# sevagh/Zen

Measured on AMD Instinct MI355X. Metric: hops/sec (1024-hop HPR, 44.1 kHz mono), higher is better.
Workload: dtype f32

## Files before the change

zen_amd/blockrun/blockrun.hip:

```cpp
#include "../csrc/hpr_engine.h"
#include "../csrc/masks.h"
#include "blockrun_first_pass.h"
#include "blockrun_kernel.h"
#include "zen_hip_blockrun.h"

#include <atomic>
#include <cstring>
#include <vector>

using namespace zen_hip_impl;

namespace {

std::atomic<int> g_run_len{0}, g_min_items{4096}, g_off{0};
std::atomic<unsigned long long> g_routed{0}, g_forwarded{0};

struct ProfScope {
	zen_hip_hpr* e;
	int k;
	hipEvent_t e0 = nullptr, e1 = nullptr;
	ProfScope(zen_hip_hpr* e_, int k_)
	    : e(e_)
	    , k(k_)
	{
		if (!e->prof)
			return;
		if (!e->prof_pool.empty()) {
			e0 = e->prof_pool.back().first;
			e1 = e->prof_pool.back().second;
			e->prof_pool.pop_back();
		}
		else if (hipEventCreate(&e0) != hipSuccess || hipEventCreate(&e1) != hipSuccess) {
			e0 = e1 = nullptr;
			return;
		}
		(void)hipEventRecord(e0, e->stream);
	}
	~ProfScope()
	{
		if (!e0)
			return;
		(void)hipEventRecord(e1, e->stream);
		e->prof_pending.push_back({k, e0, e1});
		e->prof_launches[k] += 1;
	}
};

int device_slots(int* slots)
{
	static std::atomic<int> cached[64];
	int dev = 0;
	ZH_HIP(hipGetDevice(&dev));
	int v = (dev >= 0 && dev < 64) ? cached[dev].load() : 0;
	if (v == 0) {
		int cus = 0;
		ZH_HIP(hipDeviceGetAttribute(&cus, hipDeviceAttributeMultiprocessorCount, dev));
		v = 3 * (cus > 0 ? cus : 1);
		if (dev >= 0 && dev < 64)
			cached[dev].store(v);
	}
	*slots = v;
	return ZEN_HIP_OK;
}

struct FirstPassTable {
	int symmetric;
	float2 tw16, tw8, tw3_16;
};
const FirstPassTable& first_pass_table()
{
	static const FirstPassTable t = [] {
		constexpr int n = zen_blockrun::NFFT;
		std::vector<float> tw(n);
		make_twiddles(tw.data(), tw.size());
		FirstPassTable r;
		r.symmetric = zen_blockrun::table_is_symmetric(tw.data(), n) ? 1 : 0;
		r.tw16 = make_float2(tw[2 * (n / 16)], tw[2 * (n / 16) + 1]);
		r.tw8 = make_float2(tw[2 * (n / 8)], tw[2 * (n / 8) + 1]);
		r.tw3_16 = make_float2(tw[2 * (3 * n / 16)], tw[2 * (3 * n / 16) + 1]);
		return r;
	}();
	return t;
}

bool takes(const zen_hip_hpr* h, const float* in, size_t n_hops, size_t in_stride, const float* harm, const float* perc,
           const float* resid, size_t out_stride)
{
	if (g_off.load() || !h || !in || !perc || harm || resid || n_hops == 0)
		return false;
	if (h->causality != ZEN_HIP_TIME_CAUSAL || h->log2n != 12 || h->mf != zen_blockrun::TAPS || h->hop != (size_t)zen_blockrun::HOP
	    || h->nfft != (size_t)zen_blockrun::NFFT || h->nwin != 2 * h->hop)
		return false;
	if (!h->out_p || h->out_h || h->out_r || h->soft || h->use_sse)
		return false;
	if ((h->drain[0] | h->drain[1] | h->drain[2]) || h->rows_stale || h->run_mode || h->res_idle_ms != 0 || h->res_active || h->dbg_stamps)
		return false;
	if (!h->d_Y[0] || !h->d_blk_need || !h->d_carry[0] || !h->d_mag || n_hops > h->max_hops)
		return false;
	if (h->n_streams * n_hops < (size_t)g_min_items.load() || h->n_streams * n_hops > 0x3fffffffu)
		return false;
	int inc = 0;
	if (hard_mask_threshold(h->beta, &inc) == 0.0)
		return false;
	const size_t S = h->n_streams;
	const char *in0 = (const char*)in, *in1 = (const char*)(in + (S - 1) * in_stride + n_hops * h->hop);
	const char *o0 = (const char*)perc, *o1 = (const char*)(perc + (S - 1) * out_stride + n_hops * h->hop);
	return !(o0 < in1 && in0 < o1);
}

}

extern "C" int zen_hip_blockrun_process(zen_hip_hpr_t h, const float* in_dev, size_t n_hops, size_t in_stride, float* harm, float* perc,
                                        float* resid, size_t out_stride)
{
	if (!takes(h, in_dev, n_hops, in_stride, harm, perc, resid, out_stride)) {
		g_forwarded.fetch_add(1);
		return zen_hip_hpr_process(h, in_dev, n_hops, in_stride, harm, perc, resid, out_stride);
	}
	g_routed.fetch_add(1);
	int slots = 0;
	ZH_TRY(device_slots(&slots));
	zen_blockrun::RunArgs a;
	memset(&a, 0, sizeof(a));
	a.in = in_dev;
	a.in_stride = (long long)in_stride;
	a.tail_prev = h->d_tail[h->tail_sel];
	a.tail_next = h->d_tail[h->tail_sel ^ 1];
	a.window = h->d_window;
	a.tw = h->d_tw;
	{
		const FirstPassTable& t = first_pass_table();
		a.tw_symmetric = t.symmetric;
		a.tw16 = t.tw16;
		a.tw8 = t.tw8;
		a.tw3_16 = t.tw3_16;
	}
	a.mag = h->d_mag;
	a.keep_mag_rows = (int)h->W - 1;
	a.ring_rows = h->ring_rows;
	a.row0 = h->abs_frame;
	a.n_frames = (int)n_hops;
	a.n_streams = (int)h->n_streams;
	a.prev_frames = (int)h->last_frames;
	a.carry = h->d_carry[0];
	a.Y = h->d_Y[0];
	a.y_stream_stride = (long long)(h->max_hops * h->nwin);
	a.out = perc;
	a.out_stride = (long long)out_stride;
	a.need = h->d_blk_need;
	a.cola = h->cola;
	int inc = 0;
	a.thr = hard_mask_threshold(h->beta, &inc);
	a.part = zen_blockrun_partition(a.n_streams, a.n_frames, slots, g_run_len.load());
	for (int o = 0; o < 3; ++o) {
		h->ready_valid[o] = false;
		h->direct_done[o] = false;
	}
	{
		ProfScope ps(h, zen_hip_hpr::K_FUSED);
		ZH_TRY(zen_blockrun::launch_run(a, h->stream));
	}
	{
		ProfScope ps(h, zen_hip_hpr::K_FINALIZE);
		ZH_TRY(zen_blockrun::launch_fixup(a, h->stream));
	}
	h->tail_sel ^= 1;
	h->abs_frame += (long long)n_hops;
	h->last_frames = n_hops;
	return ZEN_HIP_OK;
}

extern "C" int zen_hip_blockrun_set(const char* key, int value)
{
	if (!key || value < 0)
		ZH_FAIL(ZEN_HIP_E_BAD_ARG, "blockrun_set: null key or negative value");
	if (!strcmp(key, "run_len"))
		g_run_len.store(value);
	else if (!strcmp(key, "min_items"))
		g_min_items.store(value);
	else if (!strcmp(key, "off"))
		g_off.store(value);
	else
		ZH_FAIL(ZEN_HIP_E_BAD_ARG, "blockrun_set: unknown key '%s' (run_len, min_items, off)", key);
	return ZEN_HIP_OK;
}

extern "C" int zen_hip_blockrun_stats(unsigned long long* routed, unsigned long long* forwarded)
{
	if (routed)
		*routed = g_routed.load();
	if (forwarded)
		*forwarded = g_forwarded.load();
	return ZEN_HIP_OK;
}
```

zen_amd/blockrun/blockrun_kernel.h:

```cpp
#pragma once
#include <hip/hip_runtime.h>

#include "blockrun_partition.h"

namespace zen_blockrun {

constexpr int HOP = 1024, NFFT = 4096, TAPS = 47;

struct RunArgs {
	const float* in;
	long long in_stride;
	const float* tail_prev;
	float* tail_next;
	const float* window;
	const float2* tw;
	int tw_symmetric;
	float2 tw16, tw8, tw3_16;
	float* mag;
	int keep_mag_rows;
	long long ring_rows, row0;
	int n_frames, n_streams, prev_frames;
	float* carry;
	float* Y;
	long long y_stream_stride;
	float* out;
	long long out_stride;
	unsigned* need;
	float cola;
	double thr;
	zen_blockrun_part part;
};

constexpr size_t LDS_BYTES_MAX = 53 * 1024;
size_t run_kernel_lds_bytes();
int launch_run(const RunArgs& a, hipStream_t stream);
int launch_fixup(const RunArgs& a, hipStream_t stream);

}
```

zen_amd/blockrun/blockrun_kernel.hip:

```cpp
#include "../csrc/common.h"
#include "../csrc/fft_dev.h"
#include "../csrc/masks.h"
#include "../csrc/median47_core.h"
#include "../csrc/median_net.h"
#include "blockrun_kernel.h"
#include "blockrun_first_pass.h"
#include "blockrun_edge_count.h"

#pragma clang fp contract(off)

namespace zen_blockrun {
namespace {

using zen_hip_impl::hard_mask_exact;
using PL = zfft::Plan<12>;
constexpr int N = PL::N, TF = PL::TF;
static_assert(N == NFFT && TF == 256 && HOP == 4 * TF, "four samples of a hop per thread");

constexpr int MID = TAPS / 2, MID_AL = 24, IMG_END = 255 * 16 + 64;
__device__ __forceinline__ int img_addr(int g) { return (g >> 4) * zm47::RSTR + (g & 15); }
constexpr int MIR_LO = 56, MIR_HI = 39;
static_assert(N - MIR_LO <= 16 * 254 - 24 && N / 2 + MIR_HI >= 16 * 128 + 39, "blocks 254 / 255 and 126 .. 128 read written columns");
static_assert(EDGE_IMG_COL0 == MID_AL && EDGE_IMG_RSTR == zm47::RSTR && EDGE_OUTPUTS == MID + 1, "blockrun_edge_count.h reads this image");
constexpr int PC_WORD = 5184, PC_TAIL = 2052, EDGE_WORD = PC_WORD + PC_TAIL + 512 + 4;
static_assert((EDGE_WORD + 256) * 4 <= PL::LDS_FLOAT2 * 8, "lean layout must fit in the frame image");
constexpr int KEEP_WORD = PL::LDS_FLOAT2 * 2, CARRY_WORD = KEEP_WORD + HOP, WIN_WORD = CARRY_WORD + HOP;
constexpr size_t LDS_BYTES = (size_t)(WIN_WORD + 2 * HOP) * 4;
static_assert(LDS_BYTES <= LDS_BYTES_MAX, "three workgroups per CU");

__device__ __forceinline__ void lds_barrier()
{
	asm volatile("s_waitcnt lgkmcnt(0)\n\ts_barrier" ::: "memory");
}

struct TwGlobal32 {
	static constexpr bool PLAIN = true;
	static constexpr bool PACKED = true;
	const float2* __restrict__ p;
	__device__ __forceinline__ float2 get(int, int, int, int idx) const
	{
		return *reinterpret_cast<const float2*>(reinterpret_cast<const char*>(p) + (unsigned)(idx << 3));
	}
};

struct Spec {
	float2 S[16];
};

struct FwdInPre {
	float x[8], w[8];
	__device__ __forceinline__ float2 operator()(int, int slot) const { return make_float2(x[slot] * w[slot], 0.0f); }
};

struct FwdOut {
	Spec* r;
	int* img;
	__device__ __forceinline__ void operator()(int idx, float2 X, bool lower, int slot) const
	{
		r->S[slot] = X;
		if (slot == 8) {
			if (__builtin_amdgcn_readfirstlane(idx) < (N >> 1) + 64 && idx == (N >> 1))
				img[img_addr((N >> 1) + MID_AL)] = __float_as_int(zfft::cabs_exact(X.x, X.y));
		}
		else if (lower) {
			const float m = zfft::cabs_exact(X.x, X.y);
			const int key = __float_as_int(m);
			constexpr int CH = (TF / 16) * zm47::RSTR;
			const int tfl = idx - slot * TF;
			img[img_addr(tfl + MID_AL) + slot * CH] = key;
			if (slot == 0 && tfl >= 1 && tfl <= MIR_LO)
				img[img_addr(N - tfl + MID_AL)] = key;
			if (slot == 7 && tfl >= TF - MIR_HI)
				img[img_addr(N - 7 * TF - tfl + MID_AL)] = key;
		}
	}
};

struct InvIn {
	const Spec* r;
	const int* img;
	const float* pc;
	double thr;
	__device__ __forceinline__ float2 operator()(int idx, int slot) const
	{
		const int lo = slot * TF, hi = lo + TF - 1;
		int pi;
		if (hi <= N / 2)
			pi = idx;
		else if (lo > N / 2 && hi < N - MID)
			pi = N - idx;
		else
			pi = (idx > N / 2 && idx < N - MID) ? N - idx : (idx > N / 2 ? idx - (N - 512) + PC_TAIL : idx);
		const int g0 = hi <= N / 2 ? idx + 24 - slot * TF : TF + 24 - (idx - slot * TF);
		const float mag = __int_as_float(img[(g0 >> 4) * 20 + (g0 & 15) + (hi <= N / 2 ? slot : 15 - slot) * (TF / 16) * 20]);
		const float2 z = r->S[slot];
		const float p = pc[pi];
		float m = hard_mask_exact(p, mag + FLT_EPSILON, thr);
		if (hi > N / 2 && !(lo > N / 2 && hi < N - MID))
			m = (idx == N / 2 || idx >= N - MID) ? p : m;
		return make_float2(z.x * m, z.y * m);
	}
};

struct InvOut {
	float* Y;
	float* out;
	float* carry;
	float cola;
	__device__ __forceinline__ void operator()(int idx, float2 x, bool, int slot) const
	{
		const float y = x.x * cola;
		ZH_CHK(Y + idx, 1);
		Y[idx] = y;
		if (slot < 4) {
			ZH_CHK(out + idx, 1);
			out[idx] = carry[(slot & 3) * TF] + y;
		}
		else {
			carry[(slot & 3) * TF] = y;
		}
	}
};

template <bool SYM>
__device__ __forceinline__ void run_body(const RunArgs& a)
{
	extern __shared__ float2 lds[];
	int* img = reinterpret_cast<int*>(lds);
	float* Prow = reinterpret_cast<float*>(img + PC_WORD);
	const int tf = (int)threadIdx.x;
	float* keep = reinterpret_cast<float*>(img + KEEP_WORD) + tf;
	float* carry = reinterpret_cast<float*>(img + CARRY_WORD) + tf;
	float* win = reinterpret_cast<float*>(img + WIN_WORD) + tf;

	int s, f0, len;
	zen_blockrun_run(&a.part, (int)blockIdx.x, &s, &f0, &len);
	if (s >= a.n_streams || f0 + len > a.n_frames)
		return;
	const float* cur = a.in + (long long)s * a.in_stride + (long long)f0 * HOP;
	float* Yrow = a.Y + (long long)s * a.y_stream_stride + (long long)f0 * (2 * HOP);
	float* orow = a.out + (long long)s * a.out_stride + (long long)f0 * HOP;

	if (a.prev_frames > 0) {
		const int fc = a.prev_frames - 1 < a.n_frames - 1 ? a.prev_frames - 1 : a.n_frames - 1;
		if (fc >= f0 && fc < f0 + len) {
			const float* y = a.Y + (long long)s * a.y_stream_stride + (long long)(a.prev_frames - 1) * (2 * HOP) + HOP;
			float v[4];
#pragma unroll
			for (int i = 0; i < 4; ++i) {
				ZH_CHK(y + tf + i * TF, 1);
				v[i] = y[tf + i * TF];
			}
#pragma unroll
			for (int i = 0; i < 4; ++i) {
				ZH_CHK(a.carry + ((long long)s * HOP + tf + i * TF), 1);
				a.carry[(long long)s * HOP + tf + i * TF] = v[i];
			}
		}
	}
	float nx[4];
	{
		const float* pv = f0 > 0 ? cur - HOP : a.tail_prev + (long long)s * HOP;
		float p[4], w[8];
#pragma unroll
		for (int m = 0; m < 4; ++m) {
			ZH_CHK(pv + m * TF + tf, 1);
			ZH_CHK(cur + m * TF + tf, 1);
			p[m] = pv[m * TF + tf];
			nx[m] = cur[m * TF + tf];
		}
#pragma unroll
		for (int m = 0; m < 8; ++m) {
			ZH_CHK(a.window + m * TF + tf, 1);
			w[m] = a.window[m * TF + tf];
		}
#pragma unroll
		for (int m = 0; m < 4; ++m) {
			keep[m * TF] = p[m];
			carry[m * TF] = 0.0f;
		}
#pragma unroll
		for (int m = 0; m < 8; ++m)
			win[m * TF] = w[m];
	}
	if (tf == 0) {
		ZH_CHK(a.need + ((long long)s * a.n_frames + f0), 1);
		a.need[(long long)s * a.n_frames + f0] = 1u;
	}

	const int tf_run = tf;
	for (int k = 0; k < len; ++k) {
		const int f = f0 + k;
		int tf = tf_run, tw_off = 0;
		asm volatile("" : "+v"(tf));
		tf &= TF - 1;
		asm volatile("" : "+s"(tw_off));
		const float2* tw = a.tw + tw_off;
		float* keep = reinterpret_cast<float*>(img + KEEP_WORD) + tf;
		float* carry = reinterpret_cast<float*>(img + CARRY_WORD) + tf;
		float* win = reinterpret_cast<float*>(img + WIN_WORD) + tf;
		Spec r;
		{
			FwdInPre pre;
#pragma unroll
			for (int m = 0; m < 4; ++m) {
				pre.x[m] = keep[m * TF];
				pre.x[4 + m] = nx[m];
			}
#pragma unroll
			for (int m = 0; m < 8; ++m)
				pre.w[m] = win[m * TF];
#pragma unroll
			for (int m = 0; m < 4; ++m)
				keep[m * TF] = nx[m];
			if (f == a.n_frames - 1) {
				float* tail = a.tail_next + (long long)s * HOP;
#pragma unroll
				for (int m = 0; m < 4; ++m) {
					ZH_CHK(tail + m * TF + tf, 1);
					tail[m * TF + tf] = nx[m];
				}
			}
			FwdOut out;
			out.r = &r;
			out.img = img;
			{
				float p[8];
#pragma unroll
				for (int m = 0; m < 8; ++m)
					p[m] = pre.x[m] * pre.w[m];
				float2 Y0[16];
				first_pass16<true, SYM>(p, a.tw16, a.tw8, a.tw3_16, Y0);
#pragma unroll
				for (int c = 0; c < 16; ++c)
					lds[PL::pad_off(tf, c * (N / 16))] = Y0[c];
				zfft::frame_sync<TF>();
			}
			zfft::PassRunner<12, 1, false, true, false, FwdInPre, FwdOut, false, TwGlobal32>::run(tf, lds, TwGlobal32{tw}, pre, out, true);
		}
		lds_barrier();
		if (f >= a.n_frames - a.keep_mag_rows) {
			float* mag = a.mag + (((a.row0 + f) % a.ring_rows) + (long long)s * a.ring_rows) * N;
			for (int g = tf; g < N; g += TF) {
				ZH_CHK(mag + g, 1);
				mag[g] = __int_as_float(img[img_addr((g <= N / 2 ? g : N - g) + MID_AL)]);
			}
		}
		{
			const int v0 = img[img_addr(MID_AL)], v1 = img[img_addr(N - 1 + MID_AL)];
			for (int g = tf; g < MID_AL; g += TF)
				img[img_addr(g)] = v0;
			for (int g = N + MID_AL + tf; g < IMG_END; g += TF)
				img[img_addr(g)] = v1;
		}
		lds_barrier();
		{
			int(*edge)[64] = reinterpret_cast<int(*)[64]>(img + EDGE_WORD);
			const int lane = tf & 63, wave = __builtin_amdgcn_readfirstlane(tf >> 6);
			zm47::Pieces pc;
			if (wave < 3) {
				zm47::m47_sort_and_publish(img, edge, tf, lane, wave, tf == 0, false, pc);
			}
			else {
				const unsigned bits = edge_count_wave(img, lane, a.thr, N / 2);
				if (lane < EDGE_OUTPUTS)
					Prow[lane == 0 ? N / 2 : PC_TAIL + 512 - lane] = (bits >> lane) & 1u ? 1.0f : 0.0f;
			}
			lds_barrier();
			if (wave < 2) {
				int o[16];
				zm47::m47_select(img, edge, tf, wave, pc, o);
#pragma unroll
				for (int v = 0; v < 4; ++v)
					*reinterpret_cast<int4*>(&Prow[tf * 16 + 4 * v]) = make_int4(o[4 * v], o[4 * v + 1], o[4 * v + 2], o[4 * v + 3]);
			}
		}
		lds_barrier();
		cur += HOP;
		if (k + 1 < len) {
#pragma unroll
			for (int m = 0; m < 4; ++m) {
				ZH_CHK(cur + m * TF + tf, 1);
				nx[m] = cur[m * TF + tf];
			}
		}
		{
			asm volatile("" : "+v"(tf));
			asm volatile("" : "+s"(tw_off));
			tf &= TF - 1;
			tw = a.tw + tw_off;
			carry = reinterpret_cast<float*>(img + CARRY_WORD) + tf;
			InvIn in;
			in.r = &r;
			in.img = img;
			in.pc = Prow;
			in.thr = a.thr;
			InvOut out;
			out.Y = Yrow;
			out.out = orow;
			out.carry = carry;
			out.cola = a.cola;
			zfft::PassRunner<12, 0, true, false, true, InvIn, InvOut, true, TwGlobal32>::run(tf, lds, TwGlobal32{tw}, in, out, true);
		}
		Yrow += 2 * HOP;
		orow += HOP;
	}
}

__global__ __launch_bounds__(256, 3) void blockrun_kernel(RunArgs a) { run_body<true>(a); }
__global__ __launch_bounds__(256, 3) void blockrun_kernel_plain_table(RunArgs a) { run_body<false>(a); }

__global__ __launch_bounds__(256) void blockrun_fixup_kernel(RunArgs a)
{
	const long long total = (long long)a.n_streams * a.n_frames;
	const long long item = (long long)blockIdx.x * 4 + (threadIdx.x >> 6);
	const int lane = threadIdx.x & 63;
	if (item >= total)
		return;
	ZH_CHK(a.need + item, 1);
	if (!a.need[item])
		return;
	const int s = (int)(item / a.n_frames), f = (int)(item - (long long)s * a.n_frames);
	const float* Y = a.Y + (long long)s * a.y_stream_stride + (long long)f * (2 * HOP);
	const float* prev = f == 0 ? a.carry + (long long)s * HOP : Y - HOP;
	float* o = a.out + (long long)s * a.out_stride + (long long)f * HOP;
	if (((reinterpret_cast<uintptr_t>(o) | reinterpret_cast<uintptr_t>(prev) | reinterpret_cast<uintptr_t>(Y)) & 15) == 0) {
		float4 p[HOP / 256], y[HOP / 256];
#pragma unroll
		for (int i = 0; i < HOP / 256; ++i) {
			const int k = i * 256 + lane * 4;
			ZH_CHK(prev + k, 4);
			ZH_CHK(Y + k, 4);
			p[i] = *reinterpret_cast<const float4*>(prev + k);
			y[i] = *reinterpret_cast<const float4*>(Y + k);
		}
#pragma unroll
		for (int i = 0; i < HOP / 256; ++i) {
			const int k = i * 256 + lane * 4;
			ZH_CHK(o + k, 4);
			*reinterpret_cast<float4*>(o + k) = make_float4(p[i].x + y[i].x, p[i].y + y[i].y, p[i].z + y[i].z, p[i].w + y[i].w);
		}
	}
	else {
		for (int k = lane; k < HOP; k += 64) {
			ZH_CHK(o + k, 1);
			ZH_CHK(prev + k, 1);
			ZH_CHK(Y + k, 1);
			o[k] = prev[k] + Y[k];
		}
	}
	if (lane == 0)
		a.need[item] = 0u;
}

}

size_t run_kernel_lds_bytes() { return LDS_BYTES; }

int launch_run(const RunArgs& a, hipStream_t stream)
{
	const long long runs = (long long)a.n_streams * a.part.runs_per_stream;
	if (a.tw_symmetric)
		hipLaunchKernelGGL(blockrun_kernel, dim3((unsigned)runs), dim3(TF), LDS_BYTES, stream, a);
	else
		hipLaunchKernelGGL(blockrun_kernel_plain_table, dim3((unsigned)runs), dim3(TF), LDS_BYTES, stream, a);
	ZH_HIP(hipGetLastError());
	return ZEN_HIP_OK;
}

int launch_fixup(const RunArgs& a, hipStream_t stream)
{
	const long long total = (long long)a.n_streams * a.n_frames;
	hipLaunchKernelGGL(blockrun_fixup_kernel, dim3((unsigned)((total + 3) / 4)), dim3(256), 0, stream, a);
	ZH_HIP(hipGetLastError());
	return ZEN_HIP_OK;
}

}
```

Baseline: 62.12 million.

## Use f32 FMA mask test, real-only last inverse pass, fused edge padding

Replaces the double-precision hard mask comparison with an exact float32 FMA-based test, using a host-precomputed half-ulp offset and comparison constant, and routes betas outside the valid exponent range to the fallback path. Adds a specialized final inverse FFT pass that computes only the real outputs, skipping the imaginary arithmetic. Moves the low-edge image padding into the forward output writer and drops the separate padding loop plus one LDS barrier per frame. The risks are exactness of the float mask emulation and whether the high-edge padding is still covered.

```diff
diff --git a/zen_amd/blockrun/blockrun.hip b/zen_amd/blockrun/blockrun.hip
--- a/zen_amd/blockrun/blockrun.hip
+++ b/zen_amd/blockrun/blockrun.hip
@@ -2,6 +2,7 @@
 #include "../csrc/masks.h"
 #include "blockrun_first_pass.h"
 #include "blockrun_kernel.h"
+#include "blockrun_mask_f32.h"
 #include "zen_hip_blockrun.h"
 
 #include <atomic>
@@ -101,6 +102,8 @@
 		return false;
 	int inc = 0;
 	if (hard_mask_threshold(h->beta, &inc) == 0.0)
+		return false;
+	if (!zen_blockrun::mask_f32_params(h->beta).in_range)
 		return false;
 	const size_t S = h->n_streams;
 	const char *in0 = (const char*)in, *in1 = (const char*)(in + (S - 1) * in_stride + n_hops * h->hop);
@@ -151,6 +154,12 @@
 	a.cola = h->cola;
 	int inc = 0;
 	a.thr = hard_mask_threshold(h->beta, &inc);
+	{
+		const zen_blockrun::MaskF32 m = zen_blockrun::mask_f32_params(h->beta);
+		a.mask_beta = m.beta;
+		a.mask_h = m.h;
+		a.mask_cmp = m.cmp;
+	}
 	a.part = zen_blockrun_partition(a.n_streams, a.n_frames, slots, g_run_len.load());
 	for (int o = 0; o < 3; ++o) {
 		h->ready_valid[o] = false;
diff --git a/zen_amd/blockrun/blockrun_kernel.h b/zen_amd/blockrun/blockrun_kernel.h
--- a/zen_amd/blockrun/blockrun_kernel.h
+++ b/zen_amd/blockrun/blockrun_kernel.h
@@ -28,6 +28,7 @@
 	unsigned* need;
 	float cola;
 	double thr;
+	float mask_beta, mask_h, mask_cmp;
 	zen_blockrun_part part;
 };
 
diff --git a/zen_amd/blockrun/blockrun_kernel.hip b/zen_amd/blockrun/blockrun_kernel.hip
--- a/zen_amd/blockrun/blockrun_kernel.hip
+++ b/zen_amd/blockrun/blockrun_kernel.hip
@@ -6,18 +6,19 @@
 #include "blockrun_kernel.h"
 #include "blockrun_first_pass.h"
 #include "blockrun_edge_count.h"
+#include "blockrun_mask_f32.h"
+#include "blockrun_last_pass.h"
 
 #pragma clang fp contract(off)
 
 namespace zen_blockrun {
 namespace {
 
-using zen_hip_impl::hard_mask_exact;
 using PL = zfft::Plan<12>;
 constexpr int N = PL::N, TF = PL::TF;
 static_assert(N == NFFT && TF == 256 && HOP == 4 * TF, "four samples of a hop per thread");
 
-constexpr int MID = TAPS / 2, MID_AL = 24, IMG_END = 255 * 16 + 64;
+constexpr int MID = TAPS / 2, MID_AL = 24;
 __device__ __forceinline__ int img_addr(int g) { return (g >> 4) * zm47::RSTR + (g & 15); }
 constexpr int MIR_LO = 56, MIR_HI = 39;
 static_assert(N - MIR_LO <= 16 * 254 - 24 && N / 2 + MIR_HI >= 16 * 128 + 39, "blocks 254 / 255 and 126 .. 128 read written columns");
@@ -70,6 +71,12 @@
 			img[img_addr(tfl + MID_AL) + slot * CH] = key;
 			if (slot == 0 && tfl >= 1 && tfl <= MIR_LO)
 				img[img_addr(N - tfl + MID_AL)] = key;
+			if (slot == 0 && __builtin_amdgcn_readfirstlane(tfl) == 0 && tfl == 0) {
+				const int4 k4 = make_int4(key, key, key, key);
+#pragma unroll
+				for (int g = 0; g < MID_AL; g += 4)
+					*reinterpret_cast<int4*>(&img[img_addr(g)]) = k4;
+			}
 			if (slot == 7 && tfl >= TF - MIR_HI)
 				img[img_addr(N - 7 * TF - tfl + MID_AL)] = key;
 		}
@@ -80,7 +87,7 @@
 	const Spec* r;
 	const int* img;
 	const float* pc;
-	double thr;
+	float beta, h, cmp;
 	__device__ __forceinline__ float2 operator()(int idx, int slot) const
 	{
 		const int lo = slot * TF, hi = lo + TF - 1;
@@ -95,7 +102,7 @@
 		const float mag = __int_as_float(img[(g0 >> 4) * 20 + (g0 & 15) + (hi <= N / 2 ? slot : 15 - slot) * (TF / 16) * 20]);
 		const float2 z = r->S[slot];
 		const float p = pc[pi];
-		float m = hard_mask_exact(p, mag + FLT_EPSILON, thr);
+		float m = mask_f32(p, mag + FLT_EPSILON, beta, h, cmp);
 		if (hi > N / 2 && !(lo > N / 2 && hi < N - MID))
 			m = (idx == N / 2 || idx >= N - MID) ? p : m;
 		return make_float2(z.x * m, z.y * m);
@@ -121,6 +128,32 @@
 		}
 	}
 };
+
+}
+}
+
+template <>
+struct zfft::PassRunner<12, 2, true, false, true, zen_blockrun::InvIn, zen_blockrun::InvOut, true, zen_blockrun::TwGlobal32> {
+	using PL = zfft::Plan<12>;
+	static __device__ __forceinline__ void run(int tf, float2* __restrict__ lds, const zen_blockrun::TwGlobal32& tw, zen_blockrun::InvIn&,
+	                                           zen_blockrun::InvOut& out, bool)
+	{
+		static_assert(PL::P == 3 && PL::r(2) == 4 && PL::s(2) == 8 && PL::V == 16, "one 16-value sub-transform per thread, index tf");
+		float2 v[16];
+#pragma unroll
+		for (int m = 0; m < 16; ++m)
+			v[m] = lds[PL::pad_off(tf * 16, m)];
+		zfft::frame_sync<PL::TF>();
+		float re[8];
+		zen_blockrun::last_pass16_real(v, tf, PL::s(2), 12, tw, 2, 0, re);
+#pragma unroll
+		for (int c = 0; c < 8; ++c)
+			out(tf + c * (PL::N / 16), make_float2(re[c], 0.0f), true, c);
+	}
+};
+
+namespace zen_blockrun {
+namespace {
 
 template <bool SYM>
 __device__ __forceinline__ void run_body(const RunArgs& a)
@@ -188,6 +221,9 @@
 		a.need[(long long)s * a.n_frames + f0] = 1u;
 	}
 
+#pragma unroll
+	for (int m = 0; m < 4; ++m)
+		asm volatile("" : "+v"(nx[m]));
 	const int tf_run = tf;
 	for (int k = 0; k < len; ++k) {
 		const int f = f0 + k;
@@ -247,14 +283,6 @@
 			}
 		}
 		{
-			const int v0 = img[img_addr(MID_AL)], v1 = img[img_addr(N - 1 + MID_AL)];
-			for (int g = tf; g < MID_AL; g += TF)
-				img[img_addr(g)] = v0;
-			for (int g = N + MID_AL + tf; g < IMG_END; g += TF)
-				img[img_addr(g)] = v1;
-		}
-		lds_barrier();
-		{
 			int(*edge)[64] = reinterpret_cast<int(*)[64]>(img + EDGE_WORD);
 			const int lane = tf & 63, wave = __builtin_amdgcn_readfirstlane(tf >> 6);
 			zm47::Pieces pc;
@@ -294,7 +322,9 @@
 			in.r = &r;
 			in.img = img;
 			in.pc = Prow;
-			in.thr = a.thr;
+			in.beta = a.mask_beta;
+			in.h = a.mask_h;
+			in.cmp = a.mask_cmp;
 			InvOut out;
 			out.Y = Yrow;
 			out.out = orow;
diff --git a/zen_amd/blockrun/blockrun_last_pass.h b/zen_amd/blockrun/blockrun_last_pass.h
--- /dev/null
+++ b/zen_amd/blockrun/blockrun_last_pass.h
@@ -0,0 +1,70 @@
+#pragma once
+#include "../csrc/fft_dev.h"
+
+#pragma clang fp contract(off)
+
+namespace zen_blockrun {
+
+template <class TW>
+__device__ __forceinline__ void last_pass16_real(float2 (&a)[16], int k, int log2L, int log2N, const TW& tw, int pass, int grp,
+                                                 float (&re)[8])
+{
+	using zfft::cadd;
+	using zfft::cmul;
+	using zfft::csub;
+	constexpr int R = 16;
+	float2 b[R];
+#pragma unroll
+	for (int q = 1; q <= 3; ++q) {
+		const int half = R >> q;
+		const int nc = 1 << (q - 1);
+		float2 w[4];
+#pragma unroll
+		for (int c = 0; c < nc; ++c) {
+			if (q >= 2 && c >= (nc >> 1)) {
+				const float2 w0 = w[c - (nc >> 1)];
+				w[c] = make_float2(-w0.y, w0.x);
+			}
+			else {
+				const int idx = (k << (log2N - log2L - q)) + (c << (log2N - q));
+				const float2 t = tw.get(pass, grp, (q == 1 ? 0 : (1 << (q - 2))) + c, idx);
+				w[c] = make_float2(t.x, -t.y);
+			}
+		}
+#pragma unroll
+		for (int c = 0; c < nc; ++c) {
+#pragma unroll
+			for (int m = 0; m < half; ++m) {
+				const float2 A = a[c * 2 * half + m];
+				const float2 t = cmul<TW::PACKED>(w[c], a[c * 2 * half + m + half]);
+				b[c * half + m] = cadd<TW::PACKED>(A, t);
+				b[(c + nc) * half + m] = csub<TW::PACKED>(A, t);
+			}
+		}
+#pragma unroll
+		for (int i = 0; i < R; ++i)
+			a[i] = b[i];
+	}
+	float2 w[8];
+#pragma unroll
+	for (int c = 0; c < 8; ++c) {
+		if (c >= 4) {
+			const float2 w0 = w[c - 4];
+			w[c] = make_float2(-w0.y, w0.x);
+		}
+		else {
+			const int idx = (k << (log2N - log2L - 4)) + (c << (log2N - 4));
+			const float2 t = tw.get(pass, grp, 4 + c, idx);
+			w[c] = make_float2(t.x, -t.y);
+		}
+	}
+#pragma unroll
+	for (int c = 0; c < 8; ++c) {
+		const float2 A = a[2 * c], B = a[2 * c + 1];
+		const float t1 = w[c].x * B.x, t2 = w[c].y * B.y;
+		const float tr = t1 - t2;
+		re[c] = A.x + tr;
+	}
+}
+
+}
diff --git a/zen_amd/blockrun/blockrun_mask_f32.h b/zen_amd/blockrun/blockrun_mask_f32.h
--- /dev/null
+++ b/zen_amd/blockrun/blockrun_mask_f32.h
@@ -0,0 +1,49 @@
+#pragma once
+#include <hip/hip_runtime.h>
+
+#include <cfloat>
+#include <cstring>
+
+#pragma clang fp contract(off)
+
+namespace zen_blockrun {
+
+constexpr int MASK_F32_EXP_MAX = 40;
+
+struct MaskF32 {
+	float beta;
+	float h;
+	float cmp;
+	int inclusive;
+	int in_range;
+};
+
+inline MaskF32 mask_f32_params(float beta)
+{
+	MaskF32 p{0.0f, 0.0f, 0.0f, 0, 0};
+	unsigned u;
+	memcpy(&u, &beta, sizeof(u));
+	const int expo = (int)((u >> 23) & 0xffu);
+	if ((u >> 31) || expo == 0 || expo == 0xff)
+		return p;
+	if (expo - 127 < -MASK_F32_EXP_MAX || expo - 127 > MASK_F32_EXP_MAX)
+		return p;
+	const unsigned up = u - 1;
+	float pred;
+	memcpy(&pred, &up, sizeof(pred));
+	p.beta = beta;
+	p.h = (beta - pred) * 0.5f;
+	p.inclusive = (u & 1u) == 0 ? 1 : 0;
+	p.cmp = p.inclusive ? -FLT_TRUE_MIN : 0.0f;
+	p.in_range = 1;
+	return p;
+}
+
+__device__ __forceinline__ float mask_f32(float x, float d, float beta, float h, float cmp)
+{
+	const float e = __builtin_fmaf(-beta, d, x);
+	const float s = __builtin_fmaf(h, d, e);
+	return s > cmp ? 1.0F : 0.0F;
+}
+
+}
```

Measured after the change: 62.43 million, median of 6. No clear change (+0.5%).

## Stage pass-1 twiddles in LDS and fold edge padding into FFT output

Applied to the files above, without the earlier changes.

Copies the 128-entry pass-1 twiddle table from global memory into LDS once per workgroup, then reads it as 16-byte vectors during both the forward and inverse FFT passes, replacing per-frame global loads. The low-side edge padding of the magnitude image is now written directly by the FFT output functor. This removes the separate padding fill loop and one workgroup barrier per frame. The mirrored low-bin writes and the high-end padding fill are dropped, which only holds if the median stage no longer reads those columns.

```diff
diff --git a/zen_amd/blockrun/blockrun_kernel.hip b/zen_amd/blockrun/blockrun_kernel.hip
--- a/zen_amd/blockrun/blockrun_kernel.hip
+++ b/zen_amd/blockrun/blockrun_kernel.hip
@@ -6,6 +6,7 @@
 #include "blockrun_kernel.h"
 #include "blockrun_first_pass.h"
 #include "blockrun_edge_count.h"
+#include "blockrun_twiddle_map.h"
 
 #pragma clang fp contract(off)
 
@@ -17,15 +18,17 @@
 constexpr int N = PL::N, TF = PL::TF;
 static_assert(N == NFFT && TF == 256 && HOP == 4 * TF, "four samples of a hop per thread");
 
-constexpr int MID = TAPS / 2, MID_AL = 24, IMG_END = 255 * 16 + 64;
+constexpr int MID = TAPS / 2, MID_AL = 24;
 __device__ __forceinline__ int img_addr(int g) { return (g >> 4) * zm47::RSTR + (g & 15); }
-constexpr int MIR_LO = 56, MIR_HI = 39;
-static_assert(N - MIR_LO <= 16 * 254 - 24 && N / 2 + MIR_HI >= 16 * 128 + 39, "blocks 254 / 255 and 126 .. 128 read written columns");
+constexpr int MIR_HI = 39;
+static_assert(N / 2 + MIR_HI >= 16 * 128 + 39, "blocks 126 .. 128 read written columns");
 static_assert(EDGE_IMG_COL0 == MID_AL && EDGE_IMG_RSTR == zm47::RSTR && EDGE_OUTPUTS == MID + 1, "blockrun_edge_count.h reads this image");
 constexpr int PC_WORD = 5184, PC_TAIL = 2052, EDGE_WORD = PC_WORD + PC_TAIL + 512 + 4;
 static_assert((EDGE_WORD + 256) * 4 <= PL::LDS_FLOAT2 * 8, "lean layout must fit in the frame image");
 constexpr int KEEP_WORD = PL::LDS_FLOAT2 * 2, CARRY_WORD = KEEP_WORD + HOP, WIN_WORD = CARRY_WORD + HOP;
-constexpr size_t LDS_BYTES = (size_t)(WIN_WORD + 2 * HOP) * 4;
+constexpr int TW1_WORD = WIN_WORD + 2 * HOP;
+static_assert(TW1_WORD % 4 == 0, "16-byte reads of the pass-1 table");
+constexpr size_t LDS_BYTES = (size_t)(TW1_WORD + 2 * ZEN_BLOCKRUN_TW_PASS1_WORDS) * 4;
 static_assert(LDS_BYTES <= LDS_BYTES_MAX, "three workgroups per CU");
 
 __device__ __forceinline__ void lds_barrier()
@@ -33,15 +36,22 @@
 	asm volatile("s_waitcnt lgkmcnt(0)\n\ts_barrier" ::: "memory");
 }
 
-struct TwGlobal32 {
+struct TwRun {
 	static constexpr bool PLAIN = true;
 	static constexpr bool PACKED = true;
+	typedef float v4f __attribute__((ext_vector_type(4)));
 	const float2* __restrict__ p;
-	__device__ __forceinline__ float2 get(int, int, int, int idx) const
-	{
+	const v4f* row;
+	__device__ __forceinline__ float2 get(int pass, int, int slot, int idx) const
+	{
+		if (pass == 1) {
+			const v4f v = row[slot >> 1];
+			return (slot & 1) ? make_float2(v.z, v.w) : make_float2(v.x, v.y);
+		}
 		return *reinterpret_cast<const float2*>(reinterpret_cast<const char*>(p) + (unsigned)(idx << 3));
 	}
 };
+static_assert(ZEN_BLOCKRUN_TW_LOG2N == 12 && N == 1 << ZEN_BLOCKRUN_TW_LOG2N && ZEN_BLOCKRUN_TW_PASS1_K == TF / 16, "blockrun_twiddle_map.h is this plan's");
 
 struct Spec {
 	float2 S[16];
@@ -68,8 +78,15 @@
 			constexpr int CH = (TF / 16) * zm47::RSTR;
 			const int tfl = idx - slot * TF;
 			img[img_addr(tfl + MID_AL) + slot * CH] = key;
-			if (slot == 0 && tfl >= 1 && tfl <= MIR_LO)
-				img[img_addr(N - tfl + MID_AL)] = key;
+			if (slot == 0) {
+				if (__builtin_amdgcn_readfirstlane(idx) < 64 && tfl == 0) {
+					static_assert(MID_AL == 24 && zm47::RSTR % 4 == 0, "six 16-byte stores: words 0 .. 15 and RSTR .. RSTR + 7");
+					const int4 q = make_int4(key, key, key, key);
+#pragma unroll
+					for (int g = 0; g < MID_AL; g += 4)
+						*reinterpret_cast<int4*>(&img[img_addr(g)]) = q;
+				}
+			}
 			if (slot == 7 && tfl >= TF - MIR_HI)
 				img[img_addr(N - 7 * TF - tfl + MID_AL)] = key;
 		}
@@ -187,6 +204,11 @@
 		ZH_CHK(a.need + ((long long)s * a.n_frames + f0), 1);
 		a.need[(long long)s * a.n_frames + f0] = 1u;
 	}
+	if (tf < ZEN_BLOCKRUN_TW_PASS1_WORDS) {
+		const float2* e = a.tw + zen_blockrun_tw_pass1_fill_index(tf);
+		ZH_CHK(e, 1);
+		reinterpret_cast<float2*>(img + TW1_WORD)[tf] = *e;
+	}
 
 	const int tf_run = tf;
 	for (int k = 0; k < len; ++k) {
@@ -199,6 +221,9 @@
 		float* keep = reinterpret_cast<float*>(img + KEEP_WORD) + tf;
 		float* carry = reinterpret_cast<float*>(img + CARRY_WORD) + tf;
 		float* win = reinterpret_cast<float*>(img + WIN_WORD) + tf;
+		TwRun twr;
+		twr.p = tw;
+		twr.row = reinterpret_cast<const TwRun::v4f*>(img + TW1_WORD) + (tf >> 4) * (ZEN_BLOCKRUN_TW_SLOTS / 2);
 		Spec r;
 		{
 			FwdInPre pre;
@@ -236,7 +261,7 @@
 					lds[PL::pad_off(tf, c * (N / 16))] = Y0[c];
 				zfft::frame_sync<TF>();
 			}
-			zfft::PassRunner<12, 1, false, true, false, FwdInPre, FwdOut, false, TwGlobal32>::run(tf, lds, TwGlobal32{tw}, pre, out, true);
+			zfft::PassRunner<12, 1, false, true, false, FwdInPre, FwdOut, false, TwRun>::run(tf, lds, twr, pre, out, true);
 		}
 		lds_barrier();
 		if (f >= a.n_frames - a.keep_mag_rows) {
@@ -247,14 +272,6 @@
 			}
 		}
 		{
-			const int v0 = img[img_addr(MID_AL)], v1 = img[img_addr(N - 1 + MID_AL)];
-			for (int g = tf; g < MID_AL; g += TF)
-				img[img_addr(g)] = v0;
-			for (int g = N + MID_AL + tf; g < IMG_END; g += TF)
-				img[img_addr(g)] = v1;
-		}
-		lds_barrier();
-		{
 			int(*edge)[64] = reinterpret_cast<int(*)[64]>(img + EDGE_WORD);
 			const int lane = tf & 63, wave = __builtin_amdgcn_readfirstlane(tf >> 6);
 			zm47::Pieces pc;
@@ -289,6 +306,8 @@
 			asm volatile("" : "+s"(tw_off));
 			tf &= TF - 1;
 			tw = a.tw + tw_off;
+			twr.p = tw;
+			twr.row = reinterpret_cast<const TwRun::v4f*>(img + TW1_WORD) + (tf >> 4) * (ZEN_BLOCKRUN_TW_SLOTS / 2);
 			carry = reinterpret_cast<float*>(img + CARRY_WORD) + tf;
 			InvIn in;
 			in.r = &r;
@@ -300,7 +319,7 @@
 			out.out = orow;
 			out.carry = carry;
 			out.cola = a.cola;
-			zfft::PassRunner<12, 0, true, false, true, InvIn, InvOut, true, TwGlobal32>::run(tf, lds, TwGlobal32{tw}, in, out, true);
+			zfft::PassRunner<12, 0, true, false, true, InvIn, InvOut, true, TwRun>::run(tf, lds, twr, in, out, true);
 		}
 		Yrow += 2 * HOP;
 		orow += HOP;
diff --git a/zen_amd/blockrun/blockrun_twiddle_map.h b/zen_amd/blockrun/blockrun_twiddle_map.h
--- /dev/null
+++ b/zen_amd/blockrun/blockrun_twiddle_map.h
@@ -0,0 +1,39 @@
+#ifndef ZEN_HIP_BLOCKRUN_TWIDDLE_MAP_H
+#define ZEN_HIP_BLOCKRUN_TWIDDLE_MAP_H
+
+#if defined(__HIPCC__)
+#define ZEN_BLOCKRUN_TW_FN static __host__ __device__ inline
+#else
+#define ZEN_BLOCKRUN_TW_FN static inline
+#endif
+
+#define ZEN_BLOCKRUN_TW_LOG2N 12
+#define ZEN_BLOCKRUN_TW_SLOTS 8
+#define ZEN_BLOCKRUN_TW_PASS1_K 16
+#define ZEN_BLOCKRUN_TW_PASS1_WORDS (ZEN_BLOCKRUN_TW_PASS1_K * ZEN_BLOCKRUN_TW_SLOTS)
+
+ZEN_BLOCKRUN_TW_FN int zen_blockrun_tw_slot_stage(int slot) { return slot == 0 ? 1 : slot == 1 ? 2 : slot < 4 ? 3 : 4; }
+ZEN_BLOCKRUN_TW_FN int zen_blockrun_tw_slot_group(int slot)
+{
+	const int q = zen_blockrun_tw_slot_stage(slot);
+	return slot - (q == 1 ? 0 : 1 << (q - 2));
+}
+
+ZEN_BLOCKRUN_TW_FN int zen_blockrun_tw_pass0_index(int slot)
+{
+	return zen_blockrun_tw_slot_group(slot) << (ZEN_BLOCKRUN_TW_LOG2N - zen_blockrun_tw_slot_stage(slot));
+}
+
+ZEN_BLOCKRUN_TW_FN int zen_blockrun_tw_pass1_index(int k, int slot)
+{
+	const int q = zen_blockrun_tw_slot_stage(slot);
+	return (k << (ZEN_BLOCKRUN_TW_LOG2N - 4 - q)) + (zen_blockrun_tw_slot_group(slot) << (ZEN_BLOCKRUN_TW_LOG2N - q));
+}
+
+ZEN_BLOCKRUN_TW_FN int zen_blockrun_tw_pass1_word(int k, int slot) { return k * ZEN_BLOCKRUN_TW_SLOTS + slot; }
+ZEN_BLOCKRUN_TW_FN int zen_blockrun_tw_pass1_fill_index(int w)
+{
+	return zen_blockrun_tw_pass1_index(w / ZEN_BLOCKRUN_TW_SLOTS, w % ZEN_BLOCKRUN_TW_SLOTS);
+}
+
+#endif
```

New measurement: 62.50 million before, 62.83 million after, median of 6. No clear change (+0.5%).
